# MrTornado24/IDE-3D

Measured on AMD Instinct MI355X. Metric: 512x512 RGB+seg frames/s @96 depth samples (whole job), higher is better.
Workload: dtype f32 (3x3 convs + MLPs: fp32 operands as 3 bf16 pieces, 6 products, f32 accumulate); 1 GPU; BASELINE config 2: random-init ide3d-ffhq-64-512, G.mapping + G.synthesis (64 render -> 512, 96 samples, RGB + 19-class seg) + uint8 frames, batch 4 seeds per GPU; global_batch=4, parallelism=dp1, conv_arithmetic=bf16x6, conv_arithmetic_is_library_default=True

## Files before the change

### ide-3d_amd/csrc/raymarch.hip

```cpp
#include "common.h"
#include "triplane_tap.h"
#include "raymarch_ray.h"

namespace ide3d {

typedef float f32x4 __attribute__((ext_vector_type(4)));

template <int C, int HID>
struct RmCfg {
    static constexpr int CPL = C / 16;
    static constexpr int NF = C / 4;
    static constexpr int MT1 = HID / 16;
    static constexpr int MT2 = 2;
    static constexpr int A1 = MT1 * CPL * 64 * 4;
    static constexpr int A2 = MT2 * MT1 * 64 * 4;
    static constexpr int B0 = MT1 * 16;
    static constexpr int B1 = MT2 * 16;
    static constexpr int MLP = A1 + A2 + B0 + B1;
};

template <int C, int HID>
__device__ void stage_mlp(float* __restrict__ s, const float* __restrict__ w0, const float* __restrict__ b0,
                          const float* __restrict__ w1, const float* __restrict__ b1, int nout) {
    using K = RmCfg<C, HID>;
    float* a1 = s; float* a2 = a1 + K::A1; float* sb0 = a2 + K::A2; float* sb1 = sb0 + K::B0;
    for (int i = threadIdx.x; i < K::A1; i += blockDim.x) {
        const int e = i & 3, lane = (i >> 2) & 63, rest = i >> 8;
        const int ci = rest % K::CPL, mt = rest / K::CPL;
        const int row = 16 * mt + (lane & 15), col = 4 * ((lane >> 4) + 4 * ci) + e;
        a1[i] = w0[row * C + col];
    }
    for (int i = threadIdx.x; i < K::A2; i += blockDim.x) {
        const int e = i & 3, lane = (i >> 2) & 63, rest = i >> 8;
        const int tq = rest % K::MT1, mt = rest / K::MT1;
        const int row = 16 * mt + (lane & 15), col = 16 * tq + 4 * (lane >> 4) + e;
        a2[i] = (row < nout) ? w1[row * HID + col] : 0.f;
    }
    for (int i = threadIdx.x; i < K::B0; i += blockDim.x) sb0[i] = b0[i];
    for (int i = threadIdx.x; i < K::B1; i += blockDim.x) sb1[i] = (i < nout) ? b1[i] : 0.f;
}

typedef unsigned u32x4 __attribute__((ext_vector_type(4)));
typedef __bf16 bf16x8 __attribute__((ext_vector_type(8)));
typedef __bf16 bf16x2 __attribute__((ext_vector_type(2)));
typedef float f32x2 __attribute__((ext_vector_type(2)));

template <int C, int HID>
struct RmSplit {
    static_assert(C == 32 && HID % 32 == 0, "split MLPs: 32 input channels (one K = 32 step), hidden width a multiple of 32");
    static constexpr int MT1 = HID / 16, KH = HID / 32;
    static constexpr int A1 = MT1 * 3 * 64;
    static constexpr int A2 = 2 * KH * 3 * 64;
    static constexpr int BIAS = (MT1 + 2) * 16;
    static constexpr int BYTES = (A1 + A2) * 16 + BIAS * 4;
};

__device__ __forceinline__ void split_pair3(float a, float b, unsigned (&out)[3]) {
#pragma unroll
    for (int q = 0; q < 3; ++q) {
        const f32x2 v = {a, b};
        const bf16x2 pk = __builtin_convertvector(v, bf16x2);
        out[q] = __builtin_bit_cast(unsigned, pk);
#if defined(IDE3D_SPLIT_NO_DOT2)
        if (q < 2) { a -= __uint_as_float(out[q] << 16); b -= __uint_as_float(out[q] & 0xffff0000u); }
#else
        unsigned clo = 0x0000bf80u, chi = 0xbf800000u;
        asm volatile("" : "+s"(clo), "+s"(chi));
        const bf16x2 mlo = __builtin_bit_cast(bf16x2, clo), mhi = __builtin_bit_cast(bf16x2, chi);
        if (q < 2) { a = __builtin_amdgcn_fdot2_f32_bf16(pk, mlo, a, false); b = __builtin_amdgcn_fdot2_f32_bf16(pk, mhi, b, false); }
#endif
    }
}
__device__ __forceinline__ void split8(const float (&v)[8], u32x4 (&out)[3]) {
#pragma unroll
    for (int e = 0; e < 4; ++e) {
        unsigned pk[3];
        split_pair3(v[2 * e], v[2 * e + 1], pk);
        out[0][e] = pk[0]; out[1][e] = pk[1]; out[2][e] = pk[2];
    }
}
__device__ __forceinline__ f32x4 mfma6(const u32x4 (&a)[3], const u32x4 (&b)[3], f32x4 acc) {
#pragma unroll
    for (int sum = 2; sum >= 0; --sum)
#pragma unroll
        for (int qa = 0; qa <= sum; ++qa)
            acc = __builtin_amdgcn_mfma_f32_16x16x32_bf16(__builtin_bit_cast(bf16x8, a[qa]), __builtin_bit_cast(bf16x8, b[sum - qa]), acc, 0, 0, 0);
    return acc;
}

template <int C, int HID>
__device__ void stage_mlp_split(unsigned char* __restrict__ sm, const float* __restrict__ w0, const float* __restrict__ b0,
                                const float* __restrict__ w1, const float* __restrict__ b1, int nout) {
    using K = RmSplit<C, HID>;
    u32x4* a1 = reinterpret_cast<u32x4*>(sm);
    u32x4* a2 = a1 + K::A1;
    float* sb = reinterpret_cast<float*>(a2 + K::A2);
    for (int i = threadIdx.x; i < K::MT1 * 64; i += blockDim.x) {
        const int lane = i & 63, mt = i >> 6, g = lane >> 4, row = 16 * mt + (lane & 15);
        float v[8];
#pragma unroll
        for (int k = 0; k < 8; ++k) v[k] = w0[row * C + 16 * (k / 4) + 4 * g + k % 4];
        u32x4 pc[3];
        split8(v, pc);
#pragma unroll
        for (int q = 0; q < 3; ++q) a1[(mt * 3 + q) * 64 + lane] = pc[q];
    }
    for (int i = threadIdx.x; i < 2 * K::KH * 64; i += blockDim.x) {
        const int lane = i & 63, kh = (i >> 6) % K::KH, m2 = i / (64 * K::KH), g = lane >> 4, row = 16 * m2 + (lane & 15);
        float v[8];
#pragma unroll
        for (int k = 0; k < 8; ++k) v[k] = (row < nout) ? w1[row * HID + 16 * (2 * kh + k / 4) + 4 * g + k % 4] : 0.f;
        u32x4 pc[3];
        split8(v, pc);
#pragma unroll
        for (int q = 0; q < 3; ++q) a2[((m2 * K::KH + kh) * 3 + q) * 64 + lane] = pc[q];
    }
    for (int i = threadIdx.x; i < K::MT1 * 16; i += blockDim.x) sb[i] = b0[i];
    for (int i = threadIdx.x; i < 32; i += blockDim.x) sb[K::MT1 * 16 + i] = (i < nout) ? b1[i] : 0.f;
}

template <int C, int HID>
__device__ __forceinline__ void mlp_hidden_split(const unsigned char* __restrict__ sm, const float (&f)[C / 4], f32x4 (&h)[HID / 16]) {
    using K = RmSplit<C, HID>;
    const int lane = lane_id(), g = lane >> 4;
    const u32x4* a1 = reinterpret_cast<const u32x4*>(sm);
    const f32x4* sb0 = reinterpret_cast<const f32x4*>(sm + (K::A1 + K::A2) * 16);
    u32x4 fb[3];
    split8(f, fb);
#pragma unroll
    for (int mt = 0; mt < K::MT1; ++mt) {
        const u32x4 a[3] = {a1[(mt * 3 + 0) * 64 + lane], a1[(mt * 3 + 1) * 64 + lane], a1[(mt * 3 + 2) * 64 + lane]};
        h[mt] = mfma6(a, fb, sb0[mt * 4 + g]);
    }
#pragma unroll
    for (int mt = 0; mt < K::MT1; ++mt)
#pragma unroll
        for (int r = 0; r < 4; ++r) h[mt][r] = softplus_fast(h[mt][r]);
}

template <int C, int HID>
__device__ __forceinline__ void mlp_tile_split(const unsigned char* __restrict__ sm, const float (&f)[C / 4], f32x4 (&out)[2]) {
    using K = RmSplit<C, HID>;
    const int lane = lane_id(), g = lane >> 4;
    const u32x4* a2 = reinterpret_cast<const u32x4*>(sm) + K::A1;
    const f32x4* sb1 = reinterpret_cast<const f32x4*>(sm + (K::A1 + K::A2) * 16) + K::MT1 * 4;
    f32x4 h[K::MT1];
    mlp_hidden_split<C, HID>(sm, f, h);
    u32x4 hb[K::KH][3];
#pragma unroll
    for (int kh = 0; kh < K::KH; ++kh) {
        const float v[8] = {h[2 * kh][0], h[2 * kh][1], h[2 * kh][2], h[2 * kh][3], h[2 * kh + 1][0], h[2 * kh + 1][1], h[2 * kh + 1][2], h[2 * kh + 1][3]};
        split8(v, hb[kh]);
    }
#pragma unroll
    for (int m2 = 0; m2 < 2; ++m2) {
        f32x4 acc = sb1[m2 * 4 + g];
#pragma unroll
        for (int kh = 0; kh < K::KH; ++kh) {
            const int o = ((m2 * K::KH + kh) * 3) * 64 + lane;
            const u32x4 a[3] = {a2[o], a2[o + 64], a2[o + 128]};
            acc = mfma6(a, hb[kh], acc);
        }
        out[m2] = acc;
    }
}

template <int C, int HID>
__device__ __forceinline__ float mlp_sigma_split(const unsigned char* __restrict__ sm, const float* __restrict__ s_row, const float (&f)[C / 4]) {
    using K = RmSplit<C, HID>;
    const int g = lane_id() >> 4;
    f32x4 h[K::MT1];
    mlp_hidden_split<C, HID>(sm, f, h);
    float acc = 0.f;
#pragma unroll
    for (int mt = 0; mt < K::MT1; ++mt) {
        const f32x4 w = *reinterpret_cast<const f32x4*>(s_row + 16 * mt + 4 * g);
#pragma unroll
        for (int r = 0; r < 4; ++r) acc += w[r] * h[mt][r];
    }
    acc += __shfl_xor(acc, 16);
    acc += __shfl_xor(acc, 32);
    return acc + s_row[HID];
}

__device__ __forceinline__ int gather_sample(int lane) { return lane >> 2; }
__device__ __forceinline__ int gather_block(int lane) { return lane & 3; }

template <int NF>
__device__ __forceinline__ void to_matrix_lanes(float (&f)[NF]) {
    const int lane = lane_id();
    const int src = (((lane & 15) << 2) | (lane >> 4)) << 2;
#pragma unroll
    for (int i = 0; i < NF; ++i) f[i] = __int_as_float(__builtin_amdgcn_ds_bpermute(src, __float_as_int(f[i])));
}

template <int C> struct TapBuf { float4 v[C / 16][3][4]; };

typedef const __attribute__((address_space(1))) char* GlobalBytes;
template <class T>
__device__ __forceinline__ GlobalBytes uniform_ptr(const T* p) {
    const unsigned long long v = reinterpret_cast<unsigned long long>(p);
    const unsigned lo = __builtin_amdgcn_readfirstlane((unsigned)v), hi = __builtin_amdgcn_readfirstlane((unsigned)(v >> 32));
    return reinterpret_cast<GlobalBytes>(((unsigned long long)hi << 32) | lo);
}

__device__ __forceinline__ float4 ld4_at(GlobalBytes base, unsigned byte_off, unsigned imm) {
    typedef float v4f __attribute__((ext_vector_type(4)));
    typedef const __attribute__((address_space(1))) v4f* GlobalF4;
    const v4f v = *reinterpret_cast<GlobalF4>(base + (size_t)byte_off + imm);
    return make_float4(v[0], v[1], v[2], v[3]);
}

template <int C>
__device__ __forceinline__ void issue_taps(GlobalBytes pbc, const TapAddr (&t)[3], int g, TapBuf<C>& b, unsigned lane_extra = 0) {
    constexpr int CPL = C / 16;
    const unsigned lane_b = 16u * (unsigned)g + lane_extra;
#pragma unroll
    for (int ci = 0; ci < CPL; ++ci) {
#pragma unroll
        for (int pl = 0; pl < 3; ++pl) {
            const unsigned imm = (unsigned)(pl * C + 16 * ci) * 4u;
            b.v[ci][pl][0] = ld4_at(pbc, (unsigned)t[pl].o00 * 4u + lane_b, imm); b.v[ci][pl][1] = ld4_at(pbc, (unsigned)t[pl].o01 * 4u + lane_b, imm);
            b.v[ci][pl][2] = ld4_at(pbc, (unsigned)t[pl].o10 * 4u + lane_b, imm); b.v[ci][pl][3] = ld4_at(pbc, (unsigned)t[pl].o11 * 4u + lane_b, imm);
        }
    }
}

template <int C>
__device__ __forceinline__ void blend_taps(TapBuf<C>& b, const TapAddr (&t)[3], float (&f)[C / 4]) {
    constexpr int CPL = C / 16;
#pragma unroll
    for (int ci = 0; ci < CPL; ++ci)
#pragma unroll
        for (int pl = 0; pl < 3; ++pl)
#pragma unroll
            for (int k = 0; k < 4; ++k) asm volatile("" : "+v"(b.v[ci][pl][k].x), "+v"(b.v[ci][pl][k].y), "+v"(b.v[ci][pl][k].z), "+v"(b.v[ci][pl][k].w));
#pragma unroll
    for (int ci = 0; ci < CPL; ++ci) {
        float4 a[3];
#pragma unroll
        for (int pl = 0; pl < 3; ++pl) {
            float4 acc = make_float4(0.f, 0.f, 0.f, 0.f);
            acc = f4_fma(b.v[ci][pl][0], t[pl].w00, acc);
            acc = f4_fma(b.v[ci][pl][1], t[pl].w01, acc);
            acc = f4_fma(b.v[ci][pl][2], t[pl].w10, acc);
            acc = f4_fma(b.v[ci][pl][3], t[pl].w11, acc);
            a[pl] = acc;
        }
        f[4 * ci + 0] = (a[0].x + a[1].x) + a[2].x;
        f[4 * ci + 1] = (a[0].y + a[1].y) + a[2].y;
        f[4 * ci + 2] = (a[0].z + a[1].z) + a[2].z;
        f[4 * ci + 3] = (a[0].w + a[1].w) + a[2].w;
    }
}

template <int C>
__device__ __forceinline__ void gather_features(const float* __restrict__ pb, const TapAddr (&t)[3], int g, float (&f)[C / 4]) {
    TapBuf<C> b;
    issue_taps<C>(uniform_ptr(pb), t, g, b);
    blend_taps<C>(b, t, f);
}

template <int C, int HID>
__device__ __forceinline__ void mlp_hidden(const float* __restrict__ s, const float (&f)[C / 4], f32x4 (&h)[HID / 16]) {
    using K = RmCfg<C, HID>;
    const int lane = lane_id();
    const f32x4* a1 = reinterpret_cast<const f32x4*>(s);
    const f32x4* sb0 = reinterpret_cast<const f32x4*>(s + K::A1 + K::A2);
    const int g = lane >> 4;
#pragma unroll
    for (int mt = 0; mt < K::MT1; ++mt) h[mt] = sb0[mt * 4 + g];
#pragma unroll
    for (int ci = 0; ci < K::CPL; ++ci) {
        f32x4 w[K::MT1];
#pragma unroll
        for (int mt = 0; mt < K::MT1; ++mt) w[mt] = a1[(mt * K::CPL + ci) * 64 + lane];
#pragma unroll
        for (int e = 0; e < 4; ++e)
#pragma unroll
            for (int mt = 0; mt < K::MT1; ++mt)
                h[mt] = __builtin_amdgcn_mfma_f32_16x16x4f32(w[mt][e], f[4 * ci + e], h[mt], 0, 0, 0);
    }
#pragma unroll
    for (int mt = 0; mt < K::MT1; ++mt)
#pragma unroll
        for (int r = 0; r < 4; ++r) h[mt][r] = softplus_fast(h[mt][r]);
}

template <int C, int HID>
__device__ __forceinline__ void mlp_tile(const float* __restrict__ s, const float (&f)[C / 4], f32x4 (&out)[2]) {
    using K = RmCfg<C, HID>;
    const int lane = lane_id();
    const f32x4* a2 = reinterpret_cast<const f32x4*>(s + K::A1);
    const f32x4* sb1 = reinterpret_cast<const f32x4*>(s + K::A1 + K::A2 + K::B0);
    const int g = lane >> 4;
    f32x4 h[K::MT1];
    mlp_hidden<C, HID>(s, f, h);
#pragma unroll
    for (int mt = 0; mt < 2; ++mt) out[mt] = sb1[mt * 4 + g];
#pragma unroll
    for (int tq = 0; tq < K::MT1; ++tq) {
        const f32x4 w0 = a2[(0 * K::MT1 + tq) * 64 + lane];
        const f32x4 w1 = a2[(1 * K::MT1 + tq) * 64 + lane];
#pragma unroll
        for (int e = 0; e < 4; ++e) {
            out[0] = __builtin_amdgcn_mfma_f32_16x16x4f32(w0[e], h[tq][e], out[0], 0, 0, 0);
            out[1] = __builtin_amdgcn_mfma_f32_16x16x4f32(w1[e], h[tq][e], out[1], 0, 0, 0);
        }
    }
}

template <int C, int HID>
__device__ __forceinline__ float mlp_sigma(const float* __restrict__ s, const float* __restrict__ s_row, const float (&f)[C / 4]) {
    using K = RmCfg<C, HID>;
    const int g = lane_id() >> 4;
    f32x4 h[K::MT1];
    mlp_hidden<C, HID>(s, f, h);
    float acc = 0.f;
#pragma unroll
    for (int mt = 0; mt < K::MT1; ++mt) {
        const f32x4 w = *reinterpret_cast<const f32x4*>(s_row + 16 * mt + 4 * g);
#pragma unroll
        for (int r = 0; r < 4; ++r) acc += w[r] * h[mt][r];
    }
    acc += __shfl_xor(acc, 16);
    acc += __shfl_xor(acc, 32);
    return acc + s_row[HID];
}

__device__ __forceinline__ float seg16_excl_prod(float v, float& total) {
    const int j = lane_id() & 15;
    float incl = v;
#pragma unroll
    for (int off = 1; off < 16; off <<= 1) {
        const float o = __shfl_up(incl, off, 16);
        if (j >= off) incl *= o;
    }
    total = __shfl(incl, 15, 16);
    const float prev = __shfl_up(incl, 1, 16);
    return j == 0 ? 1.0f : prev;
}

template <int C, int HID, bool SPLIT> struct MlpBytes { static constexpr int value = RmCfg<C, HID>::MLP * 4; };
template <int C, int HID> struct MlpBytes<C, HID, true> { static constexpr int value = RmSplit<C, HID>::BYTES; };

template <int C, int HID, bool SPLIT>
__device__ __forceinline__ void stage_branch(unsigned char* sm, const float* w0, const float* b0, const float* w1, const float* b1, int nout) {
    if constexpr (SPLIT) stage_mlp_split<C, HID>(sm, w0, b0, w1, b1, nout);
    else stage_mlp<C, HID>(reinterpret_cast<float*>(sm), w0, b0, w1, b1, nout);
}
template <int C, int HID, bool SPLIT>
__device__ __forceinline__ void mlp_branch(const unsigned char* sm, const float (&f)[C / 4], f32x4 (&out)[2]) {
    if constexpr (SPLIT) mlp_tile_split<C, HID>(sm, f, out);
    else mlp_tile<C, HID>(reinterpret_cast<const float*>(sm), f, out);
}

template <bool SPLIT> struct RmWaves { static constexpr int value = SPLIT ? 8 : 4; };
template <bool SPLIT> __device__ __forceinline__ void rm_claim_half_simd() { if constexpr (SPLIT) asm volatile("" ::: "v255"); }

template <int C, int HID, bool SPLIT>
__global__ void __launch_bounds__(64 * RmWaves<SPLIT>::value, 2)
render_rays_kernel(ide3d_render_params p, int64_t rays_per_block) {
    using K = RmCfg<C, HID>;
    constexpr int NW = RmWaves<SPLIT>::value;
    rm_claim_half_simd<SPLIT>();
    extern __shared__ __attribute__((aligned(16))) float lds[];
    unsigned char* s_geo = reinterpret_cast<unsigned char*>(lds);
    unsigned char* s_tex = s_geo + MlpBytes<C, HID, SPLIT>::value;
    stage_branch<C, HID, SPLIT>(s_geo, p.geo_w0, p.geo_b0, p.geo_w1, p.geo_b1, 1 + p.seg_ch);
    stage_branch<C, HID, SPLIT>(s_tex, p.tex_w0, p.tex_b0, p.tex_w1, p.tex_b1, p.feat_ch);
    __syncthreads();

    const int lane = lane_id(), wid = __builtin_amdgcn_readfirstlane(threadIdx.x >> 6);
    const int g = lane >> 4, j = lane & 15, gl = gather_block(lane);
    const int64_t total_rays = (int64_t)p.n * p.rays_per_img;
    const int blk = xcd_remap(blockIdx.x, gridDim.x);
    const int64_t ray_begin = (int64_t)blk * rays_per_block;
    int64_t ray_end = ray_begin + rays_per_block;
    if (ray_end > total_rays) ray_end = total_rays;
    const int S = p.steps;
    const int nch = p.feat_ch + p.seg_ch;
    const int sH = (int)p.tex_stride[2], sW = (int)p.tex_stride[3];
    const float zstep = (S > 1) ? (p.z_lin[1] - p.z_lin[0]) : 0.f;

    auto tile_depth = [&](int64_t ray, int s0, float& zl, float& jl) {
        const int sl = min(s0 + gather_sample(lane), S - 1);
        zl = p.z_lin[sl];
        jl = p.jitter ? p.jitter[ray * S + sl] : 0.5f;
    };
    auto tile_taps = [&](int n, int r, float zl, float jl, TapAddr (&t)[3]) {
        float wx, wy, wz;
        ray_world_point(p, n, r, zl, jl, zstep, wx, wy, wz);
        t[0] = make_tap_addr(wx, wy, p.W, p.H, sH, sW);
        t[1] = make_tap_addr(wy, wz, p.W, p.H, sH, sW);
        t[2] = make_tap_addr(wx, wz, p.W, p.H, sH, sW);
    };

    int64_t ray = ray_begin + wid;
    int n = __builtin_amdgcn_readfirstlane((int)(ray / p.rays_per_img));
    int r = __builtin_amdgcn_readfirstlane((int)(ray - (int64_t)n * p.rays_per_img));
    int s0 = 0;
    bool have = ray < ray_end;
    TapAddr t[3];
    TapBuf<C> buf;
    if (have) {
        float zl, jl;
        tile_depth(ray, 0, zl, jl);
        tile_taps(n, r, zl, jl, t);
        issue_taps<C>(uniform_ptr(p.geo_planes + n * p.geo_stride[0]), t, gl, buf);
    }
    float acc_t[8], acc_g[8];
#pragma unroll
    for (int i = 0; i < 8; ++i) { acc_t[i] = 0.f; acc_g[i] = 0.f; }
    float carry = 1.0f, wsum = 0.f, dsum = 0.f;

    while (have) {
        int s0n = s0 + 16, nn = n, rn = r;
        int64_t rayn = ray;
        if (s0n >= S) {
            s0n = 0; rayn = ray + NW; rn = r + NW;
            while (rn >= p.rays_per_img) { rn -= (int)p.rays_per_img; ++nn; }
        }
        const bool haven = rayn < ray_end;
        const int64_t rayp = haven ? rayn : ray;
        const int np = haven ? nn : n, rp = haven ? rn : r, s0p = haven ? s0n : s0;
        const int s = s0 + j;
        const bool live = s < S;
        const int sc = live ? s : S - 1;
        float z = p.z_lin[sc];
        float znext = (sc + 1 < S) ? p.z_lin[sc + 1] : 0.f;
        if (p.jitter) {
            const float* jit = p.jitter + ray * S;
            z = __fadd_rn(z, __fmul_rn(__fsub_rn(jit[sc], 0.5f), zstep));
            if (sc + 1 < S) znext = __fadd_rn(znext, __fmul_rn(__fsub_rn(jit[sc + 1], 0.5f), zstep));
        }
        const float noise = p.sigma_noise ? p.sigma_noise[ray * S + sc] : 0.f;
        float zln, jln;
        tile_depth(rayp, s0p, zln, jln);

        float fg[K::NF], ft[K::NF];
        f32x4 og[2], ot[2];
        blend_taps<C>(buf, t, fg);
        to_matrix_lanes(fg);
        issue_taps<C>(uniform_ptr(p.tex_planes + n * p.tex_stride[0]), t, gl, buf);
        mlp_branch<C, HID, SPLIT>(s_geo, fg, og);

        float sigma = __shfl(og[0][0], j);
        sigma += noise;
        const float dens = p.clamp_mode == 0 ? softplus_fast(sigma) : fmaxf(sigma, 0.f);
        float dnorm;
        {
            const float dx = p.rays_d_cam[r * 3 + 0], dy = p.rays_d_cam[r * 3 + 1], dz = p.rays_d_cam[r * 3 + 2];
            dnorm = sqrtf(dx * dx + dy * dy + dz * dz);
        }
        const float delta = (sc + 1 < S) ? (znext - z) * dnorm : 1e10f;
        const float alpha = live ? 1.0f - __expf(-delta * dens) : 0.f;
        const float fac = live ? (1.0f - alpha + 1e-10f) : 1.0f;
        float tot;
        const float excl = seg16_excl_prod(fac, tot);
        const float w = alpha * (carry * excl);
        carry *= tot;
        wsum += w; dsum += w * z;
#pragma unroll
        for (int mt = 0; mt < 2; ++mt)
#pragma unroll
            for (int rr = 0; rr < 4; ++rr) acc_g[mt * 4 + rr] += w * og[mt][rr];

        blend_taps<C>(buf, t, ft);
        to_matrix_lanes(ft);
        tile_taps(np, rp, zln, jln, t);
        issue_taps<C>(uniform_ptr(p.geo_planes + np * p.geo_stride[0]), t, gl, buf);
        mlp_branch<C, HID, SPLIT>(s_tex, ft, ot);
#pragma unroll
        for (int mt = 0; mt < 2; ++mt)
#pragma unroll
            for (int rr = 0; rr < 4; ++rr) acc_t[mt * 4 + rr] += w * ot[mt][rr];

        if (s0n == 0) {
#pragma unroll
            for (int off = 8; off > 0; off >>= 1) {
                wsum += __shfl_xor(wsum, off); dsum += __shfl_xor(dsum, off);
#pragma unroll
                for (int i = 0; i < 8; ++i) { acc_g[i] += __shfl_xor(acc_g[i], off); acc_t[i] += __shfl_xor(acc_t[i], off); }
            }
            if (j == 0) {
                const float bg = p.white_back ? (1.0f - wsum) : 0.f;
                float* of = p.out_feat + (int64_t)n * nch * p.rays_per_img + r;
#pragma unroll
                for (int mt = 0; mt < 2; ++mt)
#pragma unroll
                    for (int rr = 0; rr < 4; ++rr) {
                        const int idx = 16 * mt + 4 * g + rr;
                        if (idx < p.feat_ch) of[(int64_t)idx * p.rays_per_img] = acc_t[mt * 4 + rr] + bg;
                        if (idx >= 1 && idx <= p.seg_ch) of[(int64_t)(p.feat_ch + idx - 1) * p.rays_per_img] = acc_g[mt * 4 + rr] + bg;
                    }
                if (g == 0) {
                    if (p.out_depth) p.out_depth[ray] = dsum + ((p.max_depth != 0.f) ? (1.0f - wsum) * p.max_depth : 0.f);
                    if (p.out_wsum) p.out_wsum[ray] = wsum;
                }
            }
#pragma unroll
            for (int i = 0; i < 8; ++i) { acc_t[i] = 0.f; acc_g[i] = 0.f; }
            carry = 1.0f; wsum = 0.f; dsum = 0.f;
        }
        ray = rayn; n = nn; r = rn; s0 = s0n; have = haven;
    }
    if constexpr (SPLIT) __syncthreads();
}

struct PointsFromMemory {
    const float* pts;
    __device__ __forceinline__ void get(int64_t row, int64_t , float& x, float& y, float& z) const {
        x = pts[row * 3 + 0]; y = pts[row * 3 + 1]; z = pts[row * 3 + 2];
    }
};

struct PointsFromLattice {
    ide3d_lattice lat;
    int64_t first;
    __device__ __forceinline__ void get(int64_t , int64_t idx, float& x, float& y, float& z) const {
        const int64_t i = first + idx;
        const float fn = (float)lat.n, fi = (float)i;
        const float q = __fdiv_rn(fi, fn);
        const int64_t r2 = (i >> 32) == 0 ? (int64_t)((unsigned)i % (unsigned)lat.n) : i % lat.n;
        const float s2 = (float)r2, s1 = fmodf(q, fn), s0 = fmodf(__fdiv_rn(q, fn), fn);
        x = __fmul_rn(__fadd_rn(__fmul_rn(s0, lat.voxel_size), lat.corner[2]), lat.scale);
        y = __fmul_rn(__fadd_rn(__fmul_rn(s1, lat.voxel_size), lat.corner[1]), lat.scale);
        z = __fmul_rn(__fadd_rn(__fmul_rn(s2, lat.voxel_size), lat.corner[0]), lat.scale);
    }
};

template <class Src>
__global__ void lattice_points_kernel(Src src, int64_t count, float* __restrict__ out) {
    for (int64_t i = (int64_t)blockIdx.x * blockDim.x + threadIdx.x; i < count; i += (int64_t)gridDim.x * blockDim.x) {
        float x, y, z;
        src.get(i, i, x, y, z);
        out[i * 3 + 0] = x; out[i * 3 + 1] = y; out[i * 3 + 2] = z;
    }
}

template <int C, int HID, class Src, bool SPLIT>
__global__ void __launch_bounds__(64 * RmWaves<SPLIT>::value, 2)
sample_voxel_kernel(ide3d_render_params p, const Src src, int64_t m, float* __restrict__ out, int64_t tiles_per_block) {
    using K = RmCfg<C, HID>;
    constexpr int NW = RmWaves<SPLIT>::value;
    rm_claim_half_simd<SPLIT>();
    extern __shared__ __attribute__((aligned(16))) float lds[];
    constexpr int MB = MlpBytes<C, HID, SPLIT>::value;
    unsigned char* s_geo = reinterpret_cast<unsigned char*>(lds);
    unsigned char* s_tex = s_geo + MB;
    float* s_stage = reinterpret_cast<float*>(s_geo + 2 * MB);
    stage_branch<C, HID, SPLIT>(s_geo, p.geo_w0, p.geo_b0, p.geo_w1, p.geo_b1, 1 + p.seg_ch);
    stage_branch<C, HID, SPLIT>(s_tex, p.tex_w0, p.tex_b0, p.tex_w1, p.tex_b1, p.feat_ch);
    __syncthreads();
    const int lane = lane_id(), wid = __builtin_amdgcn_readfirstlane(threadIdx.x >> 6);
    const int g = lane >> 4, j = lane & 15, gl = gather_block(lane);
    const int width = p.feat_ch + p.seg_ch + 1;
    const int sH = (int)p.tex_stride[2], sW = (int)p.tex_stride[3];
    float* stage = s_stage + wid * 16 * width;
    const int64_t rows = (int64_t)p.n * m;
    const int64_t ntiles = cdiv64(rows, 16);
    const int blk = xcd_remap(blockIdx.x, gridDim.x);
    const int64_t tile_begin = (int64_t)blk * tiles_per_block;
    int64_t tile_end = tile_begin + tiles_per_block;
    if (tile_end > ntiles) tile_end = ntiles;

    int64_t tile = tile_begin + wid;
    int n0 = 0;
    int64_t img_end = m;
    auto advance_image = [&](int64_t row0) { while (row0 >= img_end && n0 + 1 < p.n) { ++n0; img_end += m; } };
    auto tile_point = [&](int64_t row0, float& wx, float& wy, float& wz, int& dn) {
        const int64_t rl = row0 + gather_sample(lane);
        const int64_t rc = rl < rows ? rl : rows - 1;
        dn = 0;
        int64_t e = img_end;
        while (rc >= e) { ++dn; e += m; }
        src.get(rc, rc - (e - m), wx, wy, wz);
    };
    auto tile_taps = [&](float wx, float wy, float wz, TapAddr (&t)[3]) {
        t[0] = make_tap_addr(wx, wy, p.W, p.H, sH, sW);
        t[1] = make_tap_addr(wy, wz, p.W, p.H, sH, sW);
        t[2] = make_tap_addr(wx, wz, p.W, p.H, sH, sW);
    };
    const unsigned geo_img_b = (unsigned)p.geo_stride[0] * 4u, tex_img_b = (unsigned)p.tex_stride[0] * 4u;

    bool have = tile < tile_end;
    TapAddr t[3];
    TapBuf<C> buf;
    int dn = 0;
    if (have) {
        float wx, wy, wz;
        advance_image(tile * 16);
        tile_point(tile * 16, wx, wy, wz, dn);
        tile_taps(wx, wy, wz, t);
        issue_taps<C>(uniform_ptr(p.geo_planes + n0 * p.geo_stride[0]), t, gl, buf, (unsigned)dn * geo_img_b);
    }
    while (have) {
        const int64_t row0 = tile * 16;
        const int64_t tilen = tile + NW;
        const bool haven = tilen < tile_end;
        const int n0c = n0, dnc = dn;
        const int64_t tilep = haven ? tilen : tile;
        float wxn, wyn, wzn;
        advance_image(tilep * 16);
        tile_point(tilep * 16, wxn, wyn, wzn, dn);
        float fg[K::NF];
        blend_taps<C>(buf, t, fg);
        to_matrix_lanes(fg);
        issue_taps<C>(uniform_ptr(p.tex_planes + n0c * p.tex_stride[0]), t, gl, buf, (unsigned)dnc * tex_img_b);
        f32x4 og[2];
        mlp_branch<C, HID, SPLIT>(s_geo, fg, og);
        float ft[K::NF];
        blend_taps<C>(buf, t, ft);
        to_matrix_lanes(ft);
        tile_taps(wxn, wyn, wzn, t);
        issue_taps<C>(uniform_ptr(p.geo_planes + n0 * p.geo_stride[0]), t, gl, buf, (unsigned)dn * geo_img_b);
        f32x4 ot[2];
        mlp_branch<C, HID, SPLIT>(s_tex, ft, ot);
#pragma unroll
        for (int mt = 0; mt < 2; ++mt)
#pragma unroll
            for (int rr = 0; rr < 4; ++rr) {
                const int idx = 16 * mt + 4 * g + rr;
                if (idx < p.feat_ch) stage[j * width + idx] = ot[mt][rr];
                if (idx >= 1 && idx <= p.seg_ch) stage[j * width + p.feat_ch + idx - 1] = og[mt][rr];
                if (idx == 0) stage[j * width + width - 1] = og[mt][rr];
            }
        __builtin_amdgcn_wave_barrier();
        __builtin_amdgcn_fence(__ATOMIC_RELEASE, "wavefront");
        const int64_t live_rows = (rows - row0 < 16) ? rows - row0 : 16;
        const int64_t nel = live_rows * width;
        float* dst = out + row0 * width;
        for (int i = lane; i < nel; i += kWave) dst[i] = stage[i];
        __builtin_amdgcn_wave_barrier();
        tile = tilen; have = haven;
    }
    if constexpr (SPLIT) __syncthreads();
}

template <int C, int HID, class Src, bool SPLIT>
__global__ void __launch_bounds__(64 * RmWaves<SPLIT>::value, 2)
density_kernel(ide3d_render_params p, const Src src, int64_t m, float* __restrict__ out_sigma, int64_t supers_per_block) {
    using K = RmCfg<C, HID>;
    constexpr int NW = RmWaves<SPLIT>::value;
    rm_claim_half_simd<SPLIT>();
    extern __shared__ __attribute__((aligned(16))) float lds[];
    unsigned char* s_geo = reinterpret_cast<unsigned char*>(lds);
    float* const s_row = reinterpret_cast<float*>(s_geo + MlpBytes<C, HID, SPLIT>::value);
    stage_branch<C, HID, SPLIT>(s_geo, p.geo_w0, p.geo_b0, p.geo_w1, p.geo_b1, 1 + p.seg_ch);
    for (int i = threadIdx.x; i <= HID; i += blockDim.x) s_row[i] = (i < HID) ? p.geo_w1[i] : p.geo_b1[0];
    __syncthreads();
    const int lane = lane_id(), wid = __builtin_amdgcn_readfirstlane(threadIdx.x >> 6);
    const int g = lane >> 4, j = lane & 15, gl = gather_block(lane);
    const int sH = (int)p.geo_stride[2], sW = (int)p.geo_stride[3];
    const int64_t rows = (int64_t)p.n * m;
    const int64_t nsuper = cdiv64(rows, 64);
    const int blk = xcd_remap(blockIdx.x, gridDim.x);
    const int64_t super_begin = (int64_t)blk * supers_per_block;
    int64_t super_end = super_begin + supers_per_block;
    if (super_end > nsuper) super_end = nsuper;
    const unsigned geo_img_b = (unsigned)p.geo_stride[0] * 4u;

    int n0 = 0;
    int64_t img_end = m;
    auto super_taps = [&](int64_t st, TapAddr (&tl)[3], int& dnl) {
        const int64_t row0 = st * 64;
        while (row0 >= img_end && n0 + 1 < p.n) { ++n0; img_end += m; }
        const int64_t rl = row0 + lane;
        const int64_t rc = rl < rows ? rl : rows - 1;
        dnl = 0;
        int64_t e = img_end;
        while (rc >= e) { ++dnl; e += m; }
        float wx, wy, wz;
        src.get(rc, rc - (e - m), wx, wy, wz);
        tl[0] = make_tap_addr(wx, wy, p.W, p.H, sH, sW);
        tl[1] = make_tap_addr(wy, wz, p.W, p.H, sH, sW);
        tl[2] = make_tap_addr(wx, wz, p.W, p.H, sH, sW);
    };
    auto tile_taps = [&](const TapAddr (&tl)[3], int dnl, int k, TapAddr (&t)[3], int& dn) {
        const int src_b = (16 * k + gather_sample(lane)) << 2;
#pragma unroll
        for (int pl = 0; pl < 3; ++pl) {
            t[pl].o00 = __builtin_amdgcn_ds_bpermute(src_b, tl[pl].o00); t[pl].o01 = __builtin_amdgcn_ds_bpermute(src_b, tl[pl].o01);
            t[pl].o10 = __builtin_amdgcn_ds_bpermute(src_b, tl[pl].o10); t[pl].o11 = __builtin_amdgcn_ds_bpermute(src_b, tl[pl].o11);
            t[pl].w00 = __int_as_float(__builtin_amdgcn_ds_bpermute(src_b, __float_as_int(tl[pl].w00)));
            t[pl].w01 = __int_as_float(__builtin_amdgcn_ds_bpermute(src_b, __float_as_int(tl[pl].w01)));
            t[pl].w10 = __int_as_float(__builtin_amdgcn_ds_bpermute(src_b, __float_as_int(tl[pl].w10)));
            t[pl].w11 = __int_as_float(__builtin_amdgcn_ds_bpermute(src_b, __float_as_int(tl[pl].w11)));
        }
        dn = __builtin_amdgcn_ds_bpermute(src_b, dnl);
    };

    int64_t st = super_begin + wid;
    if (st < super_end) {
    TapAddr tl[3], t[3];
    TapBuf<C> buf;
    int dnl, dn;
    super_taps(st, tl, dnl);
    tile_taps(tl, dnl, 0, t, dn);
    issue_taps<C>(uniform_ptr(p.geo_planes + n0 * p.geo_stride[0]), t, gl, buf, (unsigned)dn * geo_img_b);
    while (st < super_end) {
        const int64_t stn = st + NW;
        const int64_t stp = stn < super_end ? stn : st;
#pragma unroll
        for (int k = 0; k < 4; ++k) {
            const int64_t row = st * 64 + 16 * k + j;
            float fg[K::NF];
            blend_taps<C>(buf, t, fg);
            to_matrix_lanes(fg);
            if (k == 3) super_taps(stp, tl, dnl);
            tile_taps(tl, dnl, (k + 1) & 3, t, dn);
            issue_taps<C>(uniform_ptr(p.geo_planes + n0 * p.geo_stride[0]), t, gl, buf, (unsigned)dn * geo_img_b);
            float sig;
            if constexpr (SPLIT) sig = mlp_sigma_split<C, HID>(s_geo, s_row, fg);
            else sig = mlp_sigma<C, HID>(reinterpret_cast<const float*>(s_geo), s_row, fg);
            if (g == 0 && row < rows) out_sigma[row] = sig;
        }
        st = stn;
    }
    }
    if constexpr (SPLIT) __syncthreads();
}

template <int C, int HID, bool SPLIT = false>
static int launch_render(const ide3d_render_params& p, hipStream_t st) {
    const size_t lds_bytes = (size_t)2 * MlpBytes<C, HID, SPLIT>::value;
    const int64_t total_rays = (int64_t)p.n * p.rays_per_img;
    constexpr int NW = RmWaves<SPLIT>::value;
    int64_t nblk = kNumCU * 8 / NW;
    int64_t rpb = cdiv64(cdiv64(total_rays, nblk), NW) * NW;
    if (rpb < NW) rpb = NW;
    nblk = cdiv64(total_rays, rpb);
    auto kern = render_rays_kernel<C, HID, SPLIT>;
    (void)hipFuncSetAttribute(reinterpret_cast<const void*>(kern), hipFuncAttributeMaxDynamicSharedMemorySize, (int)lds_bytes);
    if constexpr (SPLIT) IDE3D_EXCL_LAUNCH(kern, dim3((unsigned)nblk), 64 * NW, lds_bytes, st, p, rpb);
    else hipLaunchKernelGGL(kern, dim3((unsigned)nblk), dim3(64 * NW), lds_bytes, st, p, rpb);
    IDE3D_CHECK_LAUNCH("render_rays");
    return IDE3D_OK;
}

template <int C, int HID, class Src, bool SPLIT = false>
static int launch_voxel(const ide3d_render_params& p, const Src& src, int64_t m, float* out, float* out_sigma,
                        int sigma_only, hipStream_t st) {
    constexpr int NW = RmWaves<SPLIT>::value;
    {
        const int64_t rows_per_tile = sigma_only ? 64 : 16;
        const int64_t max_dn = (p.n > 1) ? ((rows_per_tile - 1) / (m > 0 ? m : 1) + 1 < p.n - 1 ? (rows_per_tile - 1) / (m > 0 ? m : 1) + 1 : p.n - 1) : 0;
        const int64_t img = p.geo_stride[0] > p.tex_stride[0] ? p.geo_stride[0] : p.tex_stride[0];
        if ((max_dn * img + img) * 4 >= 0xffffffffLL) { set_error("sample_voxel: too few points per image for planes this large"); return IDE3D_ENOKERNEL; }
    }
    if (sigma_only) {
        const size_t lds_bytes = (size_t)MlpBytes<C, HID, SPLIT>::value + (size_t)(HID + 4) * sizeof(float);
        const int64_t nsuper = cdiv64((int64_t)p.n * m, 64);
        int64_t nblk = kNumCU * 8 / NW;
        int64_t spb = cdiv64(cdiv64(nsuper, nblk), NW) * NW;
        if (spb < NW) spb = NW;
        nblk = cdiv64(nsuper, spb);
        auto kern = density_kernel<C, HID, Src, SPLIT>;
        (void)hipFuncSetAttribute(reinterpret_cast<const void*>(kern), hipFuncAttributeMaxDynamicSharedMemorySize, (int)lds_bytes);
        if constexpr (SPLIT) IDE3D_EXCL_LAUNCH(kern, dim3((unsigned)nblk), 64 * NW, lds_bytes, st, p, src, m, out_sigma, spb);
        else hipLaunchKernelGGL(kern, dim3((unsigned)nblk), dim3(64 * NW), lds_bytes, st, p, src, m, out_sigma, spb);
        IDE3D_CHECK_LAUNCH("sample_voxel (densities)");
        return IDE3D_OK;
    }
    const int width = p.feat_ch + p.seg_ch + 1;
    const size_t lds_bytes = (size_t)2 * MlpBytes<C, HID, SPLIT>::value + (size_t)NW * 16 * width * sizeof(float);
    const int64_t ntiles = cdiv64((int64_t)p.n * m, 16);
    int64_t nblk = kNumCU * 8 / NW;
    int64_t tpb = cdiv64(cdiv64(ntiles, nblk), NW) * NW;
    if (tpb < NW) tpb = NW;
    nblk = cdiv64(ntiles, tpb);
    auto kern = sample_voxel_kernel<C, HID, Src, SPLIT>;
    (void)hipFuncSetAttribute(reinterpret_cast<const void*>(kern), hipFuncAttributeMaxDynamicSharedMemorySize, (int)lds_bytes);
    if constexpr (SPLIT) IDE3D_EXCL_LAUNCH(kern, dim3((unsigned)nblk), 64 * NW, lds_bytes, st, p, src, m, out, tpb);
    else hipLaunchKernelGGL(kern, dim3((unsigned)nblk), dim3(64 * NW), lds_bytes, st, p, src, m, out, tpb);
    IDE3D_CHECK_LAUNCH("sample_voxel");
    return IDE3D_OK;
}

}

static bool mlp_split_selected() { return ide3d_get_conv_arithmetic() != 1; }

extern "C" int ide3d_render_rays(const ide3d_render_params* pp, void* stream) {
    using namespace ide3d;
    IDE3D_CHECK_ARG(pp != nullptr, "render_rays: null params");
    const ide3d_render_params& p = *pp;
    int rc = check_render_params(p, "render_rays", true);
    if (rc) return rc;
    if (p.last_back) { set_error("render_rays: last_back is not fused; use the step-wise ops"); return IDE3D_ENOKERNEL; }
    if (!planes_fast(p)) { set_error("render_rays: tri-planes must be channels_last, 16-byte aligned"); return IDE3D_ENOKERNEL; }
    hipStream_t st = (hipStream_t)stream;
    if (p.C == 32 && p.hidden == 64) return mlp_split_selected() ? launch_render<32, 64, true>(p, st) : launch_render<32, 64>(p, st);
    if (p.C == 16 && p.hidden == 32) return launch_render<16, 32>(p, st);
    set_error("render_rays: no fused kernel for C=%d hidden=%d", p.C, p.hidden);
    return IDE3D_ENOKERNEL;
}

extern "C" int ide3d_sample_voxel(const ide3d_render_params* pp, const float* pts, int64_t m,
                                  float* out, float* out_sigma, int sigma_only, void* stream) {
    using namespace ide3d;
    IDE3D_CHECK_ARG(pp != nullptr && pts != nullptr, "sample_voxel: null params");
    const ide3d_render_params& p = *pp;
    int rc = check_render_params(p, "sample_voxel", false);
    if (rc) return rc;
    IDE3D_CHECK_ARG(m >= 0, "sample_voxel: bad point count");
    IDE3D_CHECK_ARG(sigma_only ? out_sigma != nullptr : out != nullptr, "sample_voxel: null output");
    if (m == 0) return IDE3D_OK;
    if (!planes_fast(p)) { set_error("sample_voxel: tri-planes must be channels_last, 16-byte aligned"); return IDE3D_ENOKERNEL; }
    hipStream_t st = (hipStream_t)stream;
    const PointsFromMemory src{pts};
    if (p.C == 32 && p.hidden == 64) return mlp_split_selected() ? launch_voxel<32, 64, PointsFromMemory, true>(p, src, m, out, out_sigma, sigma_only, st)
                                                                  : launch_voxel<32, 64>(p, src, m, out, out_sigma, sigma_only, st);
    if (p.C == 16 && p.hidden == 32) return launch_voxel<16, 32>(p, src, m, out, out_sigma, sigma_only, st);
    set_error("sample_voxel: no fused kernel for C=%d hidden=%d", p.C, p.hidden);
    return IDE3D_ENOKERNEL;
}

static int check_lattice(const ide3d_lattice* lat, int64_t first, int64_t count, const char* what) {
    using namespace ide3d;
    IDE3D_CHECK_ARG(lat != nullptr && lat->n >= 2 && lat->n <= 2048, "%s: lattice resolution must be in [2, 2048]", what);
    const int64_t total = (int64_t)lat->n * lat->n * lat->n;
    IDE3D_CHECK_ARG(first >= 0 && count >= 0 && first + count <= total, "%s: point range outside the lattice", what);
    return IDE3D_OK;
}

extern "C" int ide3d_lattice_points(const ide3d_lattice* lat, int64_t first, int64_t count, float* pts, void* stream) {
    using namespace ide3d;
    int rc = check_lattice(lat, first, count, "lattice_points");
    if (rc) return rc;
    IDE3D_CHECK_ARG(pts != nullptr || count == 0, "lattice_points: null output");
    if (count == 0) return IDE3D_OK;
    const PointsFromLattice src{*lat, first};
    hipLaunchKernelGGL(lattice_points_kernel<PointsFromLattice>, dim3(stream_grid(count, 256)), dim3(256), 0, (hipStream_t)stream,
                       src, count, pts);
    IDE3D_CHECK_LAUNCH("lattice_points");
    return IDE3D_OK;
}

extern "C" int ide3d_density_lattice(const ide3d_render_params* pp, const ide3d_lattice* lat, int64_t first, int64_t count,
                                     float* out_sigma, void* stream) {
    using namespace ide3d;
    IDE3D_CHECK_ARG(pp != nullptr, "density_lattice: null params");
    const ide3d_render_params& p = *pp;
    int rc = check_render_params(p, "density_lattice", false);
    if (rc) return rc;
    rc = check_lattice(lat, first, count, "density_lattice");
    if (rc) return rc;
    IDE3D_CHECK_ARG(out_sigma != nullptr || count == 0, "density_lattice: null output");
    if (count == 0) return IDE3D_OK;
    if (!planes_fast(p)) { set_error("density_lattice: tri-planes must be channels_last, 16-byte aligned"); return IDE3D_ENOKERNEL; }
    hipStream_t st = (hipStream_t)stream;
    const PointsFromLattice src{*lat, first};
    if (p.C == 32 && p.hidden == 64) return mlp_split_selected() ? launch_voxel<32, 64, PointsFromLattice, true>(p, src, count, nullptr, out_sigma, 1, st)
                                                                  : launch_voxel<32, 64>(p, src, count, nullptr, out_sigma, 1, st);
    if (p.C == 16 && p.hidden == 32) return launch_voxel<16, 32>(p, src, count, nullptr, out_sigma, 1, st);
    set_error("density_lattice: no fused kernel for C=%d hidden=%d", p.C, p.hidden);
    return IDE3D_ENOKERNEL;
}

namespace ide3d {
const char* raymarch_build_flags() {
    return ""
#ifdef IDE3D_SPLIT_NO_DOT2
        "IDE3D_SPLIT_NO_DOT2 "
#endif
        ;
}
}
```

Before: 942.2 frames/s.

## Defer second MLP layer to per-ray after volume-rendering accumulation

Result: faster. 957.5 frames/s, median of 6 (+1.6%).

```diff
diff --git a/ide-3d_amd/csrc/raymarch.hip b/ide-3d_amd/csrc/raymarch.hip
--- a/ide-3d_amd/csrc/raymarch.hip
+++ b/ide-3d_amd/csrc/raymarch.hip
@@ -19,6 +19,17 @@
     static constexpr int MLP = A1 + A2 + B0 + B1;
 };
 
+template <int HID>
+__device__ __forceinline__ void stage_out_fp32(float* __restrict__ a2, const float* __restrict__ w1, int nout) {
+    constexpr int MT1 = HID / 16;
+    for (int i = threadIdx.x; i < 2 * MT1 * 64 * 4; i += blockDim.x) {
+        const int e = i & 3, lane = (i >> 2) & 63, rest = i >> 8;
+        const int tq = rest % MT1, mt = rest / MT1;
+        const int row = 16 * mt + (lane & 15), col = 16 * tq + 4 * (lane >> 4) + e;
+        a2[i] = (row < nout) ? w1[row * HID + col] : 0.f;
+    }
+}
+
 template <int C, int HID>
 __device__ void stage_mlp(float* __restrict__ s, const float* __restrict__ w0, const float* __restrict__ b0,
                           const float* __restrict__ w1, const float* __restrict__ b1, int nout) {
@@ -30,12 +41,7 @@
         const int row = 16 * mt + (lane & 15), col = 4 * ((lane >> 4) + 4 * ci) + e;
         a1[i] = w0[row * C + col];
     }
-    for (int i = threadIdx.x; i < K::A2; i += blockDim.x) {
-        const int e = i & 3, lane = (i >> 2) & 63, rest = i >> 8;
-        const int tq = rest % K::MT1, mt = rest / K::MT1;
-        const int row = 16 * mt + (lane & 15), col = 16 * tq + 4 * (lane >> 4) + e;
-        a2[i] = (row < nout) ? w1[row * HID + col] : 0.f;
-    }
+    stage_out_fp32<HID>(a2, w1, nout);
     for (int i = threadIdx.x; i < K::B0; i += blockDim.x) sb0[i] = b0[i];
     for (int i = threadIdx.x; i < K::B1; i += blockDim.x) sb1[i] = (i < nout) ? b1[i] : 0.f;
 }
@@ -89,22 +95,32 @@
 }
 
 template <int C, int HID>
+__device__ __forceinline__ void stage_split_layer1(u32x4* __restrict__ a1, const float* __restrict__ w0) {
+    using K = RmSplit<C, HID>;
+    for (int i = threadIdx.x; i < K::MT1 * 64; i += blockDim.x) {
+        const int lane = i & 63, mt = i >> 6, g = lane >> 4, row = 16 * mt + (lane & 15);
+        float v[8];
+#pragma unroll
+        for (int k = 0; k < 8; ++k) v[k] = w0[row * C + 16 * (k / 4) + 4 * g + k % 4];
+        u32x4 pc[3];
+        split8(v, pc);
+#pragma unroll
+        for (int q = 0; q < 3; ++q) a1[(mt * 3 + q) * 64 + lane] = pc[q];
+    }
+}
+template <int HID>
+__device__ __forceinline__ void stage_split_biases(float* __restrict__ sb, const float* __restrict__ b0, const float* __restrict__ b1, int nout) {
+    for (int i = threadIdx.x; i < HID; i += blockDim.x) sb[i] = b0[i];
+    for (int i = threadIdx.x; i < 32; i += blockDim.x) sb[HID + i] = (i < nout) ? b1[i] : 0.f;
+}
+
+template <int C, int HID>
 __device__ void stage_mlp_split(unsigned char* __restrict__ sm, const float* __restrict__ w0, const float* __restrict__ b0,
                                 const float* __restrict__ w1, const float* __restrict__ b1, int nout) {
     using K = RmSplit<C, HID>;
     u32x4* a1 = reinterpret_cast<u32x4*>(sm);
     u32x4* a2 = a1 + K::A1;
-    float* sb = reinterpret_cast<float*>(a2 + K::A2);
-    for (int i = threadIdx.x; i < K::MT1 * 64; i += blockDim.x) {
-        const int lane = i & 63, mt = i >> 6, g = lane >> 4, row = 16 * mt + (lane & 15);
-        float v[8];
-#pragma unroll
-        for (int k = 0; k < 8; ++k) v[k] = w0[row * C + 16 * (k / 4) + 4 * g + k % 4];
-        u32x4 pc[3];
-        split8(v, pc);
-#pragma unroll
-        for (int q = 0; q < 3; ++q) a1[(mt * 3 + q) * 64 + lane] = pc[q];
-    }
+    stage_split_layer1<C, HID>(a1, w0);
     for (int i = threadIdx.x; i < 2 * K::KH * 64; i += blockDim.x) {
         const int lane = i & 63, kh = (i >> 6) % K::KH, m2 = i / (64 * K::KH), g = lane >> 4, row = 16 * m2 + (lane & 15);
         float v[8];
@@ -115,16 +131,15 @@
 #pragma unroll
         for (int q = 0; q < 3; ++q) a2[((m2 * K::KH + kh) * 3 + q) * 64 + lane] = pc[q];
     }
-    for (int i = threadIdx.x; i < K::MT1 * 16; i += blockDim.x) sb[i] = b0[i];
-    for (int i = threadIdx.x; i < 32; i += blockDim.x) sb[K::MT1 * 16 + i] = (i < nout) ? b1[i] : 0.f;
-}
-
-template <int C, int HID>
+    stage_split_biases<HID>(reinterpret_cast<float*>(a2 + K::A2), b0, b1, nout);
+}
+
+template <int C, int HID, int A2U = RmSplit<C, HID>::A2>
 __device__ __forceinline__ void mlp_hidden_split(const unsigned char* __restrict__ sm, const float (&f)[C / 4], f32x4 (&h)[HID / 16]) {
     using K = RmSplit<C, HID>;
     const int lane = lane_id(), g = lane >> 4;
     const u32x4* a1 = reinterpret_cast<const u32x4*>(sm);
-    const f32x4* sb0 = reinterpret_cast<const f32x4*>(sm + (K::A1 + K::A2) * 16);
+    const f32x4* sb0 = reinterpret_cast<const f32x4*>(sm + (K::A1 + A2U) * 16);
     u32x4 fb[3];
     split8(f, fb);
 #pragma unroll
@@ -165,15 +180,12 @@
     }
 }
 
-template <int C, int HID>
-__device__ __forceinline__ float mlp_sigma_split(const unsigned char* __restrict__ sm, const float* __restrict__ s_row, const float (&f)[C / 4]) {
-    using K = RmSplit<C, HID>;
+template <int HID>
+__device__ __forceinline__ float sigma_row0(const float* __restrict__ s_row, const f32x4 (&h)[HID / 16]) {
     const int g = lane_id() >> 4;
-    f32x4 h[K::MT1];
-    mlp_hidden_split<C, HID>(sm, f, h);
     float acc = 0.f;
 #pragma unroll
-    for (int mt = 0; mt < K::MT1; ++mt) {
+    for (int mt = 0; mt < HID / 16; ++mt) {
         const f32x4 w = *reinterpret_cast<const f32x4*>(s_row + 16 * mt + 4 * g);
 #pragma unroll
         for (int r = 0; r < 4; ++r) acc += w[r] * h[mt][r];
@@ -181,6 +193,13 @@
     acc += __shfl_xor(acc, 16);
     acc += __shfl_xor(acc, 32);
     return acc + s_row[HID];
+}
+
+template <int C, int HID>
+__device__ __forceinline__ float mlp_sigma_split(const unsigned char* __restrict__ sm, const float* __restrict__ s_row, const float (&f)[C / 4]) {
+    f32x4 h[HID / 16];
+    mlp_hidden_split<C, HID>(sm, f, h);
+    return sigma_row0<HID>(s_row, h);
 }
 
 __device__ __forceinline__ int gather_sample(int lane) { return lane >> 2; }
@@ -312,20 +331,9 @@
 
 template <int C, int HID>
 __device__ __forceinline__ float mlp_sigma(const float* __restrict__ s, const float* __restrict__ s_row, const float (&f)[C / 4]) {
-    using K = RmCfg<C, HID>;
-    const int g = lane_id() >> 4;
-    f32x4 h[K::MT1];
+    f32x4 h[HID / 16];
     mlp_hidden<C, HID>(s, f, h);
-    float acc = 0.f;
-#pragma unroll
-    for (int mt = 0; mt < K::MT1; ++mt) {
-        const f32x4 w = *reinterpret_cast<const f32x4*>(s_row + 16 * mt + 4 * g);
-#pragma unroll
-        for (int r = 0; r < 4; ++r) acc += w[r] * h[mt][r];
-    }
-    acc += __shfl_xor(acc, 16);
-    acc += __shfl_xor(acc, 32);
-    return acc + s_row[HID];
+    return sigma_row0<HID>(s_row, h);
 }
 
 __device__ __forceinline__ float seg16_excl_prod(float v, float& total) {
@@ -353,6 +361,66 @@
 __device__ __forceinline__ void mlp_branch(const unsigned char* sm, const float (&f)[C / 4], f32x4 (&out)[2]) {
     if constexpr (SPLIT) mlp_tile_split<C, HID>(sm, f, out);
     else mlp_tile<C, HID>(reinterpret_cast<const float*>(sm), f, out);
+}
+
+template <int C, int HID, bool SPLIT> struct RmRender {
+    using K = RmCfg<C, HID>;
+    static constexpr int W2_OFF = K::A1 * 4, B1_OFF = (K::A1 + K::A2 + K::B0) * 4, BYTES = K::MLP * 4;
+    static constexpr int ROW = HID + 4;
+};
+template <int C, int HID> struct RmRender<C, HID, true> {
+    using K = RmSplit<C, HID>;
+    static constexpr int W2 = 2 * K::MT1 * 64;
+    static constexpr int W2_OFF = K::A1 * 16, B1_OFF = (K::A1 + W2) * 16 + HID * 4, BYTES = (K::A1 + W2) * 16 + K::BIAS * 4;
+    static constexpr int ROW = HID + 4;
+};
+
+template <int C, int HID, bool SPLIT>
+__device__ __forceinline__ void stage_render_branch(unsigned char* sm, const float* w0, const float* b0, const float* w1, const float* b1, int nout) {
+    if constexpr (SPLIT) {
+        using R = RmRender<C, HID, true>;
+        stage_split_layer1<C, HID>(reinterpret_cast<u32x4*>(sm), w0);
+        stage_out_fp32<HID>(reinterpret_cast<float*>(sm + R::W2_OFF), w1, nout);
+        stage_split_biases<HID>(reinterpret_cast<float*>(sm + R::W2_OFF + R::W2 * 16), b0, b1, nout);
+    } else {
+        stage_mlp<C, HID>(reinterpret_cast<float*>(sm), w0, b0, w1, b1, nout);
+    }
+}
+template <int C, int HID, bool SPLIT>
+__device__ __forceinline__ void hidden_branch(const unsigned char* sm, const float (&f)[C / 4], f32x4 (&h)[HID / 16]) {
+    if constexpr (SPLIT) mlp_hidden_split<C, HID, RmRender<C, HID, true>::W2>(sm, f, h);
+    else mlp_hidden<C, HID>(reinterpret_cast<const float*>(sm), f, h);
+}
+
+template <int CTRL>
+__device__ __forceinline__ float dpp_add(float v) {
+    return v + __int_as_float(__builtin_amdgcn_update_dpp(0, __float_as_int(v), CTRL, 0xf, 0xf, false));
+}
+__device__ __forceinline__ float row16_sum(float v) {
+    v = dpp_add<0xB1>(v); v = dpp_add<0x4E>(v); v = dpp_add<0x141>(v); v = dpp_add<0x140>(v);
+    return v;
+}
+
+template <int C, int HID, bool SPLIT>
+__device__ __forceinline__ void heads_per_ray(const unsigned char* sm, const float (&acc)[HID / 4], float wsum, float (&out)[2]) {
+    using R = RmRender<C, HID, SPLIT>;
+    constexpr int MT1 = HID / 16;
+    const int lane = lane_id();
+    const f32x4* w2 = reinterpret_cast<const f32x4*>(sm + R::W2_OFF);
+    const float* sb1 = reinterpret_cast<const float*>(sm + R::B1_OFF);
+#pragma unroll
+    for (int m2 = 0; m2 < 2; ++m2) {
+        float a = 0.f;
+#pragma unroll
+        for (int mt = 0; mt < MT1; ++mt) {
+            const f32x4 w = w2[(m2 * MT1 + mt) * 64 + lane];
+#pragma unroll
+            for (int r = 0; r < 4; ++r) a = fmaf(w[r], acc[4 * mt + r], a);
+        }
+        a += __shfl_xor(a, 16);
+        a += __shfl_xor(a, 32);
+        out[m2] = fmaf(sb1[16 * m2 + (lane & 15)], wsum, a);
+    }
 }
 
 template <bool SPLIT> struct RmWaves { static constexpr int value = SPLIT ? 8 : 4; };
@@ -365,10 +433,14 @@
     constexpr int NW = RmWaves<SPLIT>::value;
     rm_claim_half_simd<SPLIT>();
     extern __shared__ __attribute__((aligned(16))) float lds[];
+    using R = RmRender<C, HID, SPLIT>;
+    constexpr int NA = HID / 4;
     unsigned char* s_geo = reinterpret_cast<unsigned char*>(lds);
-    unsigned char* s_tex = s_geo + MlpBytes<C, HID, SPLIT>::value;
-    stage_branch<C, HID, SPLIT>(s_geo, p.geo_w0, p.geo_b0, p.geo_w1, p.geo_b1, 1 + p.seg_ch);
-    stage_branch<C, HID, SPLIT>(s_tex, p.tex_w0, p.tex_b0, p.tex_w1, p.tex_b1, p.feat_ch);
+    unsigned char* s_tex = s_geo + R::BYTES;
+    float* const s_row = reinterpret_cast<float*>(s_tex + R::BYTES);
+    stage_render_branch<C, HID, SPLIT>(s_geo, p.geo_w0, p.geo_b0, p.geo_w1, p.geo_b1, 1 + p.seg_ch);
+    stage_render_branch<C, HID, SPLIT>(s_tex, p.tex_w0, p.tex_b0, p.tex_w1, p.tex_b1, p.feat_ch);
+    for (int i = threadIdx.x; i <= HID; i += blockDim.x) s_row[i] = (i < HID) ? p.geo_w1[i] : p.geo_b1[0];
     __syncthreads();
 
     const int lane = lane_id(), wid = __builtin_amdgcn_readfirstlane(threadIdx.x >> 6);
@@ -409,9 +481,9 @@
         tile_taps(n, r, zl, jl, t);
         issue_taps<C>(uniform_ptr(p.geo_planes + n * p.geo_stride[0]), t, gl, buf);
     }
-    float acc_t[8], acc_g[8];
-#pragma unroll
-    for (int i = 0; i < 8; ++i) { acc_t[i] = 0.f; acc_g[i] = 0.f; }
+    float acc_t[NA], acc_g[NA];
+#pragma unroll
+    for (int i = 0; i < NA; ++i) { acc_t[i] = 0.f; acc_g[i] = 0.f; }
     float carry = 1.0f, wsum = 0.f, dsum = 0.f;
 
     while (have) {
@@ -439,13 +511,13 @@
         tile_depth(rayp, s0p, zln, jln);
 
         float fg[K::NF], ft[K::NF];
-        f32x4 og[2], ot[2];
+        f32x4 hg[K::MT1], ht[K::MT1];
         blend_taps<C>(buf, t, fg);
         to_matrix_lanes(fg);
         issue_taps<C>(uniform_ptr(p.tex_planes + n * p.tex_stride[0]), t, gl, buf);
-        mlp_branch<C, HID, SPLIT>(s_geo, fg, og);
-
-        float sigma = __shfl(og[0][0], j);
+        hidden_branch<C, HID, SPLIT>(s_geo, fg, hg);
+
+        float sigma = sigma_row0<HID>(s_row, hg);
         sigma += noise;
         const float dens = p.clamp_mode == 0 ? softplus_fast(sigma) : fmaxf(sigma, 0.f);
         float dnorm;
@@ -462,45 +534,44 @@
         carry *= tot;
         wsum += w; dsum += w * z;
 #pragma unroll
-        for (int mt = 0; mt < 2; ++mt)
-#pragma unroll
-            for (int rr = 0; rr < 4; ++rr) acc_g[mt * 4 + rr] += w * og[mt][rr];
+        for (int mt = 0; mt < K::MT1; ++mt)
+#pragma unroll
+            for (int rr = 0; rr < 4; ++rr) acc_g[mt * 4 + rr] += w * hg[mt][rr];
 
         blend_taps<C>(buf, t, ft);
         to_matrix_lanes(ft);
         tile_taps(np, rp, zln, jln, t);
         issue_taps<C>(uniform_ptr(p.geo_planes + np * p.geo_stride[0]), t, gl, buf);
-        mlp_branch<C, HID, SPLIT>(s_tex, ft, ot);
-#pragma unroll
-        for (int mt = 0; mt < 2; ++mt)
-#pragma unroll
-            for (int rr = 0; rr < 4; ++rr) acc_t[mt * 4 + rr] += w * ot[mt][rr];
+        hidden_branch<C, HID, SPLIT>(s_tex, ft, ht);
+#pragma unroll
+        for (int mt = 0; mt < K::MT1; ++mt)
+#pragma unroll
+            for (int rr = 0; rr < 4; ++rr) acc_t[mt * 4 + rr] += w * ht[mt][rr];
 
         if (s0n == 0) {
-#pragma unroll
-            for (int off = 8; off > 0; off >>= 1) {
-                wsum += __shfl_xor(wsum, off); dsum += __shfl_xor(dsum, off);
-#pragma unroll
-                for (int i = 0; i < 8; ++i) { acc_g[i] += __shfl_xor(acc_g[i], off); acc_t[i] += __shfl_xor(acc_t[i], off); }
-            }
-            if (j == 0) {
+            wsum = row16_sum(wsum); dsum = row16_sum(dsum);
+#pragma unroll
+            for (int i = 0; i < NA; ++i) { acc_g[i] = row16_sum(acc_g[i]); acc_t[i] = row16_sum(acc_t[i]); }
+            float o_t[2], o_g[2];
+            heads_per_ray<C, HID, SPLIT>(s_tex, acc_t, wsum, o_t);
+            heads_per_ray<C, HID, SPLIT>(s_geo, acc_g, wsum, o_g);
+            {
                 const float bg = p.white_back ? (1.0f - wsum) : 0.f;
                 float* of = p.out_feat + (int64_t)n * nch * p.rays_per_img + r;
-#pragma unroll
-                for (int mt = 0; mt < 2; ++mt)
-#pragma unroll
-                    for (int rr = 0; rr < 4; ++rr) {
-                        const int idx = 16 * mt + 4 * g + rr;
-                        if (idx < p.feat_ch) of[(int64_t)idx * p.rays_per_img] = acc_t[mt * 4 + rr] + bg;
-                        if (idx >= 1 && idx <= p.seg_ch) of[(int64_t)(p.feat_ch + idx - 1) * p.rays_per_img] = acc_g[mt * 4 + rr] + bg;
-                    }
-                if (g == 0) {
+                const int idx = j + 16 * (g & 1);
+                const float v = (g & 2) ? ((g & 1) ? o_g[1] : o_g[0]) : ((g & 1) ? o_t[1] : o_t[0]);
+                if (g < 2) {
+                    if (idx < p.feat_ch) of[(int64_t)idx * p.rays_per_img] = v + bg;
+                } else {
+                    if (idx >= 1 && idx <= p.seg_ch) of[(int64_t)(p.feat_ch + idx - 1) * p.rays_per_img] = v + bg;
+                }
+                if (lane == 0) {
                     if (p.out_depth) p.out_depth[ray] = dsum + ((p.max_depth != 0.f) ? (1.0f - wsum) * p.max_depth : 0.f);
                     if (p.out_wsum) p.out_wsum[ray] = wsum;
                 }
             }
 #pragma unroll
-            for (int i = 0; i < 8; ++i) { acc_t[i] = 0.f; acc_g[i] = 0.f; }
+            for (int i = 0; i < NA; ++i) { acc_t[i] = 0.f; acc_g[i] = 0.f; }
             carry = 1.0f; wsum = 0.f; dsum = 0.f;
         }
         ray = rayn; n = nn; r = rn; s0 = s0n; have = haven;
@@ -724,7 +795,8 @@
 
 template <int C, int HID, bool SPLIT = false>
 static int launch_render(const ide3d_render_params& p, hipStream_t st) {
-    const size_t lds_bytes = (size_t)2 * MlpBytes<C, HID, SPLIT>::value;
+    using R = RmRender<C, HID, SPLIT>;
+    const size_t lds_bytes = (size_t)2 * R::BYTES + (size_t)R::ROW * sizeof(float);
     const int64_t total_rays = (int64_t)p.n * p.rays_per_img;
     constexpr int NW = RmWaves<SPLIT>::value;
     int64_t nblk = kNumCU * 8 / NW;
```
